# ParaGroup/WindFlow

Hardware: NVIDIA H100
Metric: tuples/sec, Map_GPU->Filter_GPU->Ffat_Windows_GPU (CB win 4096 slide 64) pipeline (higher is better)
Workload: dtype i64+f64

## Files before the change

windflow_b200/csrc/wfb_kernels.cuh:

```cuda
#pragma once
#include <type_traits>
#include <cstdint>
#include <cstring>
#include <cuda.h>
#include <cuda_runtime.h>
#include "wfb_ptx.cuh"
#include "wfb_keys.cuh"

namespace wfb {

template <class P> using key_codec = KeyCodec<typename P::key_t>;
template <class P> using key_words_t = typename key_codec<P>::words_t;
template <class P>
__host__ __device__ __forceinline__ key_words_t<P> key_words(const typename P::tuple_t &t, const typename P::params_t &prm)
{
    return key_codec<P>::encode(P::key(t, prm));
}

constexpr int TILE = 256;
constexpr uint32_t OSW_TILE_POS = 4096;
#ifndef WFB_STAGES
#define WFB_STAGES 4
#endif
constexpr int STAGES = WFB_STAGES;
// ... 410 lines not shown
    auto stage_aux = [&](uint32_t s) { return smem + s * SM::stage_bytes + SM::tile_bytes; };

    if (tid == 0) {
        for (int s = 0; s < SM::stages; s++) { mbar_init(&full[s], 1); mbar_init(&staged[s], TILE / 32); mbar_init(&empty[s], 1); }
        mbar_fence_init();
    }
    if constexpr (MODE == MODE_INGEST) { for (uint32_t i = tid; i < 4u * 256u; i += TP_THREADS) s_hist[i] = 0; }
    __syncthreads();

    if (warp == 0) {
        if (lane == 0) {
            const uint64_t pol_first = l2_policy_evict_first();
            DevBatch b = a.one; uint32_t bi = 0, b_end = 0;
            bool have_batch = false;
            const uint32_t tpt = a.tiles_per_ticket ? a.tiles_per_ticket : 1u;
            uint32_t t_next = 0, t_end = 0, claim = 0;
            for (uint32_t it = 0;; it++) {
                const uint32_t s = it % SM::stages, par = (it / SM::stages) & 1u;
                mbar_wait(&empty[s], par ^ 1u);
                StageMeta &m = meta[s];
                if (t_next == t_end) {
                    claim = atomicAdd(a.ticket, 1u) - a.ticket_base;
                    t_next = claim * tpt;
                    if (claim >= (a.num_tiles + tpt - 1) / tpt) { m.tile = TILE_SENTINEL; mbar_arrive(&full[s]); break; }
                    t_end = min(t_next + tpt, a.num_tiles);
                }
                const uint32_t t = t_next++;
                if (a.batches != nullptr && !(have_batch && t >= b.tile_begin && t < b_end)) {
                    uint32_t lo = 0, hi = a.nbatches - 1;
                    while (lo < hi) { const uint32_t mid = (lo + hi + 1) >> 1; if (a.batches[mid].tile_begin <= t) lo = mid; else hi = mid - 1; }
                    bi = lo; b = a.batches[lo];
                    b_end = (lo + 1 < a.nbatches) ? a.batches[lo + 1].tile_begin : a.num_tiles;
                    have_batch = true;
                }
                const uint32_t first = (t - b.tile_begin) * TILE;
                const uint32_t cnt = min(static_cast<uint32_t>(TILE), b.n - first);
                const unsigned char *src = b.tuples + static_cast<size_t>(first) * TB;
                uint32_t flags = 0, tx = 0;
                const uint64_t off = reinterpret_cast<uint64_t>(src) - a.tmap_base;
                if (CAN_SWZ && a.use_tmap && cnt == TILE && (off & 63u) == 0 && (off >> 6) < 0x7fffff00ull) flags = TF_SWZ;
                else if (!bulk_ok(src, cnt * TB)) flags = TF_FALLBACK;
                if (!(flags & TF_FALLBACK)) tx += cnt * TB;
                const uint64_t *tsp = ((MODE == MODE_FILTER || MODE == MODE_FLATMAP) && b.ts != nullptr) ? b.ts + first : nullptr;
                if (tsp != nullptr && bulk_ok(tsp, cnt * 8u)) { flags |= TF_TS_SMEM; tx += cnt * 8u; }
                if (t_next == t_end) flags |= TF_WIDE_LAST;
                m.tile = t; m.batch = bi; m.first = first; m.cnt = cnt; m.flags = flags; m.wide = claim;
                if (tx) mbar_expect_tx(&full[s], tx); else mbar_arrive(&full[s]);
// ... 545 lines not shown
        if (c.z) atomicAdd(ctl_counts + tid * 4 + 2, c.z);
        if (c.w) atomicAdd(ctl_counts + tid * 4 + 3, c.w);
    }
}

static __global__ void __launch_bounds__(OSW_THREADS) k_wide_chunk_sums16(const uint16_t *__restrict__ H, uint32_t tiles, uint32_t chunk_shift, uint32_t *__restrict__ C,
                                                                          uint32_t *__restrict__ ctl_counts = nullptr)
{
    const uint32_t chunk = blockIdx.x, tid = threadIdx.x;
    const uint32_t t0 = chunk << chunk_shift, t1 = min(tiles, t0 + (1u << chunk_shift));
    uint4 acc = make_uint4(0, 0, 0, 0);
    const ushort4 *row = reinterpret_cast<const ushort4 *>(H) + tid;
#pragma unroll 16
    for (uint32_t t = t0; t < t1; t++) { const ushort4 v = row[static_cast<size_t>(t) * (OSW_DIGITS / 4)]; acc.x += v.x; acc.y += v.y; acc.z += v.z; acc.w += v.w; }
    reinterpret_cast<uint4 *>(C + static_cast<size_t>(chunk) * OSW_DIGITS)[tid] = acc;
    if (ctl_counts != nullptr) {
        if (acc.x) atomicAdd(ctl_counts + tid * 4 + 0, acc.x);
        if (acc.y) atomicAdd(ctl_counts + tid * 4 + 1, acc.y);
        if (acc.z) atomicAdd(ctl_counts + tid * 4 + 2, acc.z);
        if (acc.w) atomicAdd(ctl_counts + tid * 4 + 3, acc.w);
    }
}

static __global__ void __launch_bounds__(OSW_THREADS) k_wide_tile_bases(const uint16_t *__restrict__ H, uint32_t tiles, uint32_t chunk_shift, uint32_t chunks,
                                                                        uint32_t *__restrict__ C, uint32_t *__restrict__ T, uint32_t *__restrict__ ctl_counts,
                                                                        uint32_t *__restrict__ done, uint32_t gshift)
{
    static_assert(OSW_THREADS * 4 == OSW_DIGITS, "four digits per thread");
    constexpr uint32_t NW = OSW_THREADS / 32;
    __shared__ uint32_t wsum[NW];
    __shared__ uint32_t s_last;
    const uint32_t chunk = blockIdx.x, tid = threadIdx.x, lane = tid & 31, warp = tid >> 5;
    const uint32_t t0 = chunk << chunk_shift, t1 = min(tiles, t0 + (1u << chunk_shift));
    uint4 acc = make_uint4(0, 0, 0, 0);
    const ushort4 *row = reinterpret_cast<const ushort4 *>(H) + tid;
    uint4 *trow = reinterpret_cast<uint4 *>(T) + tid;
#pragma unroll 8
    for (uint32_t t = t0; t < t1; t++) {
        const ushort4 v = row[static_cast<size_t>(t) * (OSW_DIGITS / 4)];
        if ((t & ((1u << gshift) - 1u)) == 0) trow[static_cast<size_t>(t >> gshift) * (OSW_DIGITS / 4)] = acc;
        acc.x += v.x; acc.y += v.y; acc.z += v.z; acc.w += v.w;
    }
    uint4 *C4 = reinterpret_cast<uint4 *>(C);
    C4[static_cast<size_t>(chunk) * (OSW_DIGITS / 4) + tid] = acc;
    __threadfence();
    __syncthreads();
    if (tid == 0) s_last = atomicAdd(done, 1u) == chunks - 1u;
    __syncthreads();
    if (!s_last) return;
    __threadfence();
    uint4 tot = make_uint4(0, 0, 0, 0);
#pragma unroll 8
    for (uint32_t c = 0; c < chunks; c++) { const uint4 v = __ldcg(C4 + static_cast<size_t>(c) * (OSW_DIGITS / 4) + tid); tot.x += v.x; tot.y += v.y; tot.z += v.z; tot.w += v.w; }
    reinterpret_cast<uint4 *>(ctl_counts)[tid] = tot;
    const uint32_t sum = tot.x + tot.y + tot.z + tot.w;
    uint32_t incl = sum;
#pragma unroll
    for (int o = 1; o < 32; o <<= 1) { const uint32_t v = __shfl_up_sync(FULL, incl, o); if (lane >= static_cast<uint32_t>(o)) incl += v; }
    if (lane == 31) wsum[warp] = incl;
    __syncthreads();
    uint32_t base = incl - sum;
#pragma unroll
    for (uint32_t q = 0; q < NW; q++) if (q < warp) base += wsum[q];
    uint4 run = make_uint4(base, base + tot.x, base + tot.x + tot.y, base + tot.x + tot.y + tot.z);
#pragma unroll 8
    for (uint32_t c = 0; c < chunks; c++) {
        uint4 *p = C4 + static_cast<size_t>(c) * (OSW_DIGITS / 4) + tid;
        const uint4 v = __ldcg(p);
        *p = run;
        run.x += v.x; run.y += v.y; run.z += v.z; run.w += v.w;
    }
    if (tid == 0) *done = 0;
}

constexpr uint32_t OSR_SMEM = OSR_GROUP_POS * 2u * 2u + OSW_DIGITS * 8u + OSW_DIGITS * 2u;
static_assert(OSR_GROUP == 4 && OSR_GROUP_POS <= 0x8000u, "one ushort4 of part sizes per digit; 16-bit packed position compare");
static __global__ void __launch_bounds__(OSW_THREADS, 3) k_wide_scatter_ranked(const uint32_t *__restrict__ packed, uint32_t *__restrict__ list_out,
                                                                            uint32_t n, uint32_t shift, uint32_t chunk_shift,
                                                                            uint32_t tiles, const uint16_t *__restrict__ H, const uint32_t *__restrict__ Cx,
                                                                            const uint32_t *__restrict__ T)
{
    constexpr uint32_t NW = OSW_THREADS / 32;
    static_assert(OSW_THREADS * 4 == OSW_DIGITS, "four digits per thread");
    extern __shared__ __align__(16) unsigned char osr_smem_buf[];
    uint16_t *lpos = reinterpret_cast<uint16_t *>(osr_smem_buf);
    uint16_t *lslot = lpos + OSR_GROUP_POS;
    ushort4 *part = reinterpret_cast<ushort4 *>(lslot + OSR_GROUP_POS);
    uint16_t *cell = reinterpret_cast<uint16_t *>(part + OSW_DIGITS);
    __shared__ uint32_t wsum[NW];
    __shared__ uint32_t s_total;
    const uint32_t tid = threadIdx.x, lane = tid & 31, warp = tid >> 5, group = blockIdx.x, tile0 = group * OSR_GROUP;
    const uint32_t start = tile0 * OSW_TILE;
    if (start >= n) return;
    {
        ushort4 h[OSR_GROUP];
#pragma unroll
        for (uint32_t k = 0; k < OSR_GROUP; k++)
            h[k] = tile0 + k < tiles ? reinterpret_cast<const ushort4 *>(H)[static_cast<size_t>(tile0 + k) * (OSW_DIGITS / 4) + tid] : make_ushort4(0, 0, 0, 0);
        part[4 * tid + 0] = make_ushort4(h[0].x, h[1].x, h[2].x, h[3].x);
        part[4 * tid + 1] = make_ushort4(h[0].y, h[1].y, h[2].y, h[3].y);
        part[4 * tid + 2] = make_ushort4(h[0].z, h[1].z, h[2].z, h[3].z);
        part[4 * tid + 3] = make_ushort4(h[0].w, h[1].w, h[2].w, h[3].w);
        uint32_t c0 = 0, c1 = 0, c2 = 0, c3 = 0;
#pragma unroll
        for (uint32_t k = 0; k < OSR_GROUP; k++) { c0 += h[k].x; c1 += h[k].y; c2 += h[k].z; c3 += h[k].w; }
        const uint32_t sum = c0 + c1 + c2 + c3;
        uint32_t incl = sum;
#pragma unroll
        for (int o = 1; o < 32; o <<= 1) { const uint32_t v = __shfl_up_sync(FULL, incl, o); if (lane >= static_cast<uint32_t>(o)) incl += v; }
        if (lane == 31) wsum[warp] = incl;
        __syncthreads();
        uint32_t base = incl - sum;
#pragma unroll
        for (uint32_t q = 0; q < NW; q++) if (q < warp) base += wsum[q];
        if (tid == OSW_THREADS - 1) s_total = base + sum;
// ... 44 lines not shown
    }
}

#ifndef WFB_OSR_MINBLOCKS
#define WFB_OSR_MINBLOCKS 6
#endif
template <int RBYTES>
static __global__ void __launch_bounds__(OSW_THREADS, WFB_OSR_MINBLOCKS) k_wide_scatter_ranked_tile(const uint32_t *__restrict__ packed, uint32_t *__restrict__ keys_out,
                                                                            uint32_t list, uint32_t n, uint32_t shift, uint32_t chunk_shift,
                                                                            const uint16_t *__restrict__ H, const uint32_t *__restrict__ Cx, const uint32_t *__restrict__ T,
                                                                            const unsigned char *__restrict__ payload_in, unsigned char *__restrict__ payload_out)
{
    constexpr uint32_t NW = OSW_THREADS / 32;
    constexpr uint32_t LPOS = OSW_TILE + OSW_DIGITS;
    constexpr uint32_t LPAD = 0x0fffu;
    static_assert(OSW_TILE <= 4096 && LPOS % (2 * OSW_THREADS) == 0, "16-bit packed position compare");
    __shared__ __align__(16) uint32_t sw[OSW_TILE];
    __shared__ __align__(16) uint32_t bin_base[OSW_DIGITS];
    __shared__ __align__(8) uint16_t cnt_row[OSW_DIGITS], cell_start[OSW_DIGITS];
    __shared__ __align__(4) uint16_t lpos[LPOS];
    __shared__ uint32_t wsum[NW];
    const uint32_t tid = threadIdx.x, lane = tid & 31, warp = tid >> 5, tile = blockIdx.x;
    const uint32_t start = tile * OSW_TILE;
    if (start >= n) return;
#pragma unroll
    for (uint32_t r = 0; r < OSW_ITEMS; r++) {
        const uint32_t i = r * OSW_THREADS + tid, idx = start + i;
        const uint32_t w = idx < n ? packed[idx] : INVALID_SLOT;
        sw[i] = w;
        if constexpr (RBYTES != 0)
            if (w != INVALID_SLOT) asm volatile("prefetch.global.L2 [%0];" ::"l"(payload_in + static_cast<size_t>(idx) * RBYTES));
    }
    {
        const uint4 cb = reinterpret_cast<const uint4 *>(Cx)[static_cast<size_t>(tile >> chunk_shift) * (OSW_DIGITS / 4) + tid];
        const uint4 tb = reinterpret_cast<const uint4 *>(T)[static_cast<size_t>(tile) * (OSW_DIGITS / 4) + tid];
        reinterpret_cast<uint4 *>(bin_base)[tid] = make_uint4(cb.x + tb.x, cb.y + tb.y, cb.z + tb.z, cb.w + tb.w);
        const ushort4 c = reinterpret_cast<const ushort4 *>(H)[static_cast<size_t>(tile) * (OSW_DIGITS / 4) + tid];
        reinterpret_cast<ushort4 *>(cnt_row)[tid] = c;
        const uint32_t p0 = (c.x + 1u) & ~1u, p1 = (c.y + 1u) & ~1u, p2 = (c.z + 1u) & ~1u, p3 = (c.w + 1u) & ~1u;
        const uint32_t sum = p0 + p1 + p2 + p3;
        uint32_t incl = sum;
#pragma unroll
        for (int o = 1; o < 32; o <<= 1) { const uint32_t v = __shfl_up_sync(FULL, incl, o); if (lane >= static_cast<uint32_t>(o)) incl += v; }
        if (lane == 31) wsum[warp] = incl;
#pragma unroll
        for (uint32_t i = 0; i < LPOS / (2 * OSW_THREADS); i++) reinterpret_cast<uint32_t *>(lpos)[i * OSW_THREADS + tid] = LPAD | (LPAD << 16);
// ... 549 lines not shown
    __shared__ uint32_t s_idx[CAP];
    __shared__ uint32_t s_list[CAP];
    __shared__ __align__(16) uint16_t s_col[BK_KEYS][CS];
    __shared__ uint32_t kcnt[BK_KEYS], koff[BK_KEYS];
    __shared__ uint32_t kleft[BK_KEYS];
    __shared__ uint32_t kcp[BK_KEYS], kleaf[BK_KEYS];
    __shared__ uint64_t kc[BK_KEYS], kg[BK_KEYS], ktt[BK_KEYS];
    __shared__ __align__(16) unsigned char kacc[BK_KEYS * RB];
    __shared__ __align__(16) unsigned char s_sib[LAZY ? 16 : BK_KEYS * BK_SIBL * RB];
    __shared__ uint32_t s_heavy[BK_KEYS];
    __shared__ uint32_t ksegb[BK_KEYS];
    __shared__ uint32_t seg_desc[BK_THREADS];
    __shared__ uint32_t misc[NW], s_boff[2], s_nheavy, s_hnext, s_nseg;

    const uint32_t tid = threadIdx.x, lane = tid & 31, warp = tid >> 5;
    const uint32_t bucket = blockIdx.x;
    const uint32_t kpc = min(BK_KEYS, 1u << shift);
    const uint32_t key_lo = bucket << shift;
    const uint32_t n = ff.n_leaves, logn = ff.log_leaves;
    const uint32_t P32 = static_cast<uint32_t>(ff.pane);
    const uint64_t group_items = ff.slide * ff.nb;
    const size_t tree_stride = static_cast<size_t>(2 * n - 1) * RB;
    BK_TRACE_STATE;

    BK_MARK(0);
    uint32_t my_total = 0;
    uint64_t st_c = 0;
    const bool has_key = tid < kpc && key_lo + tid < ff.max_keys;
    if (has_key) {
        const uint32_t slot = key_lo + tid;
        st_c = ff.cnt[slot];
#pragma unroll
        for (uint32_t q = 0; q < RB / CPB; q++) cp_async<CPB>(kacc + tid * RB + q * CPB, ff.acc + static_cast<size_t>(slot) * RB + q * CPB);
    }
    if (tid < BK_KEYS) kleft[tid] = 0;
    {
        uint32_t cc[DPT];
#pragma unroll
        for (uint32_t q = 0; q < DPT / 4; q++) {
            const uint4 v = reinterpret_cast<const uint4 *>(digit_counts)[tid * (DPT / 4) + q];
            cc[4 * q] = v.x; cc[4 * q + 1] = v.y; cc[4 * q + 2] = v.z; cc[4 * q + 3] = v.w;
        }
        uint32_t sum = 0;
#pragma unroll
        for (uint32_t q = 0; q < DPT; q++) sum += cc[q];
        uint32_t incl = sum;
// ... 373 lines not shown
        uint32_t range = (ws == 0) ? n : (ws & (0u - ws));
        const uint32_t pw = 1u << (31 - __clz(remaining));
        range = min(range, pw);
        const uint32_t level = 31 - __clz(range);
        alignas(16) R node;
        ld_rec<R>(tree + static_cast<size_t>(level_off(n, level) + (ws >> level)) * RB, node);
        P::comb(res, node, res, prm);
        ws = (ws + range) & (n - 1);
        remaining -= range;
    }
    if (opos < out_cap) {
        st_rec<R>(out_res + static_cast<size_t>(opos) * RB, res);
        if (out_ts != nullptr) out_ts[opos] = wm;
    } else atomicOr(ff.err_flags, 2u);
}

template <class P>
__global__ void __launch_bounds__(256) k_ffat_windows(const FfatDev ff, const uint32_t *__restrict__ batch_off,
                                                      const DevBatch *__restrict__ batches, uint32_t nbatches,
                                                      unsigned char *__restrict__ out_res, uint64_t *__restrict__ out_ts, uint32_t out_cap,
                                                      const typename P::params_t prm, uint32_t *__restrict__ n_out)
{
    using R = typename P::result_t;
    if (blockIdx.x == 0 && threadIdx.x == 0 && n_out != nullptr) {
        if (*n_out > out_cap) { *n_out = out_cap; atomicOr(ff.err_flags, 2u); }
        if (ff.results_total != nullptr) *ff.results_total += *n_out;
    }
    const uint32_t nt = min(*ff.n_trig, ff.trig_cap);
    const uint64_t total = static_cast<uint64_t>(nt) * ff.nb;
    const size_t tree_stride = static_cast<size_t>(2 * ff.n_leaves - 1) * sizeof(R);
    for (uint64_t w = blockIdx.x * static_cast<uint64_t>(blockDim.x) + threadIdx.x; w < total; w += static_cast<uint64_t>(gridDim.x) * blockDim.x) {
        const uint32_t ti = static_cast<uint32_t>(w / ff.nb), i = static_cast<uint32_t>(w % ff.nb);
        const Trigger tr = ff.trig[ti];
        const uint64_t wm = batch_watermark(batch_off, batches, nbatches, tr.last_pos);
        ffat_eval_window<P>(ff, ff.tree + static_cast<size_t>(tr.slot) * tree_stride, trig_key<P>(ff, tr), tr.g * ff.nb + i, wm, tr.obase + i,
                            out_res, out_ts, out_cap, prm);
    }
}

template <class P>
__global__ void __launch_bounds__(128) k_ffat_windows_lazy(const FfatDev ff, const uint32_t *__restrict__ batch_off,
                                                           const DevBatch *__restrict__ batches, uint32_t nbatches,
                                                           unsigned char *__restrict__ out_res, uint64_t *__restrict__ out_ts, uint32_t out_cap,
                                                           const typename P::params_t prm, uint32_t *__restrict__ n_out)
{
    using R = typename P::result_t;
    constexpr uint32_t RB = sizeof(R);
    extern __shared__ __align__(16) unsigned char lazy_smem[];
    if (blockIdx.x == 0 && threadIdx.x == 0 && n_out != nullptr) {
        if (*n_out > out_cap) { *n_out = out_cap; atomicOr(ff.err_flags, 2u); }
        if (ff.results_total != nullptr) *ff.results_total += *n_out;
    }
    const uint32_t lane = threadIdx.x & 31, warp = threadIdx.x >> 5, wpb = blockDim.x >> 5;
    const uint32_t n = ff.n_leaves, logn = ff.log_leaves;
    unsigned char *t = lazy_smem + static_cast<size_t>(warp) * 2u * n * RB;
    const uint32_t nt = min(*ff.n_trig, ff.trig_cap);
    const size_t tree_stride = static_cast<size_t>(2 * n - 1) * RB;
    FfatDev fs = ff; fs.lazy = 0;
    for (uint32_t ti = blockIdx.x * wpb + warp; ti < nt; ti += gridDim.x * wpb) {
        const Trigger tr = ff.trig[ti];
        const unsigned char *leaves = ff.tree + static_cast<size_t>(tr.slot) * tree_stride;
        for (uint32_t i = lane; i < n * (RB / 8); i += 32) reinterpret_cast<uint64_t *>(t)[i] = reinterpret_cast<const uint64_t *>(leaves)[i];
        __syncwarp();
        for (uint32_t l = 0; l < logn; l++) {
            const unsigned char *src = t + static_cast<size_t>(level_off(n, l)) * RB;
            unsigned char *dst = t + static_cast<size_t>(level_off(n, l + 1)) * RB;
            for (uint32_t i = lane; i < (n >> (l + 1)); i += 32) {
                alignas(16) R a, b, o;
                ld_rec<R>(src + static_cast<size_t>(2 * i) * RB, a); ld_rec<R>(src + static_cast<size_t>(2 * i + 1) * RB, b);
                o = a;
                P::comb(a, b, o, prm);
// ... 1043 lines not shown
```

windflow_b200/csrc/wfb_launch.cuh:

```cuda
#pragma once
#include <type_traits>
#include <algorithm>
#include <cstring>
#include <cuda.h>
#include <cuda_runtime.h>
#include "../../include/wfb200.h"
#include "wfb_kernels.cuh"

#define WFB_CK(call) do { cudaError_t e__ = (call); if (e__ != cudaSuccess) return static_cast<int>(e__); } while (0)

namespace wfb {

inline int num_sms()
{
    static int n = 0;
    if (n == 0) { int dev = 0; if (cudaGetDevice(&dev) == cudaSuccess) cudaDeviceGetAttribute(&n, cudaDevAttrMultiProcessorCount, dev); }
    return n;
}


typedef CUresult (*PFN_encodeTiled)(CUtensorMap *, CUtensorMapDataType, cuuint32_t, void *, const cuuint64_t *, const cuuint64_t *,
                                    const cuuint32_t *, const cuuint32_t *, CUtensorMapInterleave, CUtensorMapSwizzle,
                                    CUtensorMapL2promotion, CUtensorMapFloatOOBfill);
inline PFN_encodeTiled get_encode_tiled()
{
    static PFN_encodeTiled fn = nullptr;
    static bool tried = false;
    if (!tried) {
        tried = true;
        void *p = nullptr;
        cudaDriverEntryPointQueryResult q;
        if (cudaGetDriverEntryPoint("cuTensorMapEncodeTiled", &p, cudaEnableDefault, &q) == cudaSuccess && q == cudaDriverEntryPointSuccess)
            fn = reinterpret_cast<PFN_encodeTiled>(p);
        cudaGetLastError();
    }
    return fn;
}

inline bool make_tuple_tmap(CUtensorMap *m, uint64_t base, uint64_t end)
{
// ... 114 lines not shown
    }
    return WFB_E_BADARG;
}

template <class P>
int ffat_update_dispatch(const FfatDev &ff, const unsigned char *lifted, const uint32_t *sorted_pos, const uint32_t *batch_off,
                         const DevBatch *batches, uint32_t nbatches, unsigned char *out_res, uint64_t *out_ts,
                         uint32_t out_cap, uint32_t *n_out, uint32_t grid, cudaStream_t s, const void *params, uint32_t lanes_grid)
{
    const typename P::params_t prm = load_params<P>(params);
    k_ffat_update_lanes<P><<<lanes_grid, 128, 0, s>>>(ff, lifted, sorted_pos, batch_off, batches, nbatches, out_res, out_ts, out_cap, n_out, prm);
    k_ffat_update<P><<<std::max(1u, std::min(grid, static_cast<uint32_t>(wfb::num_sms()) * 2u)), 256, 0, s>>>(
        ff, lifted, sorted_pos, batch_off, batches, nbatches, out_res, out_ts, out_cap, n_out, prm);
    WFB_CK(cudaGetLastError());
    return 0;
}

template <class P>
int ffat_buckets_dispatch(const FfatDev &ff, const unsigned char *lifted, const uint32_t *bk_list, uint32_t pos_base,
                          const uint32_t *digit_counts, uint32_t shift, uint32_t moved, const uint32_t *batch_off, const DevBatch *batches,
                          uint32_t nbatches, unsigned char *out_res, uint64_t *out_ts, uint32_t out_cap, uint32_t *n_out, cudaStream_t s,
                          const void *params)
{
    if (ff.lazy) k_ffat_update_buckets<P, true><<<OSW_DIGITS, BK_THREADS, 0, s>>>(ff, lifted, bk_list, pos_base, digit_counts, shift, moved, batch_off, batches,
                                                                                 nbatches, out_res, out_ts, out_cap, n_out, load_params<P>(params));
    else k_ffat_update_buckets<P, false><<<OSW_DIGITS, BK_THREADS, 0, s>>>(ff, lifted, bk_list, pos_base, digit_counts, shift, moved, batch_off, batches,
                                                                          nbatches, out_res, out_ts, out_cap, n_out, load_params<P>(params));
    WFB_CK(cudaGetLastError());
    return 0;
}
template <class P>
constexpr decltype(ProgramOps::ffat_buckets) ffat_buckets_of()
{
    if constexpr (bk_fits<sizeof(typename P::result_t)>()) return &ffat_buckets_dispatch<P>; else return nullptr;
}

template <class P>
int ffat_windows_dispatch(const FfatDev &ff, const uint32_t *batch_off, const DevBatch *batches, uint32_t nbatches,
                          unsigned char *out_res, uint64_t *out_ts, uint32_t out_cap, uint32_t grid, cudaStream_t s, const void *params, uint32_t *n_out)
{
    if (ff.lazy) {
        const size_t per_warp = static_cast<size_t>(2) * ff.n_leaves * sizeof(typename P::result_t);
        const uint32_t wpb = static_cast<uint32_t>(std::max<size_t>(1, std::min<size_t>(4, (32u << 10) / per_warp)));
        k_ffat_windows_lazy<P><<<grid, 32 * wpb, wpb * per_warp, s>>>(ff, batch_off, batches, nbatches, out_res, out_ts, out_cap, load_params<P>(params), n_out);
    } else
    k_ffat_windows<P><<<grid, 256, 0, s>>>(ff, batch_off, batches, nbatches, out_res, out_ts, out_cap, load_params<P>(params), n_out);
    WFB_CK(cudaGetLastError());
    return 0;
}

inline uint32_t grid_for(uint32_t n, uint32_t per_block) { return std::max(1u, std::min((n + per_block - 1) / per_block, static_cast<uint32_t>(wfb::num_sms()) * 16u)); }

template <class P>
int extract_keys_dispatch(const unsigned char *tuples, uint32_t n, uint64_t *keys, uint32_t *dest, uint32_t num_shards, cudaStream_t s,
                          const void *params)
{
    k_extract_keys<P><<<grid_for(n, 256), 256, 0, s>>>(tuples, n, keys, dest, num_shards, load_params<P>(params));
    WFB_CK(cudaGetLastError());
    return 0;
}
template <class P>
int reduce_segments_dispatch(const unsigned char *tuples, const uint64_t *ts, const uint32_t *sidx, const uint32_t *seg_begin,
                             const uint32_t *n_keys, unsigned char *out_tuples, uint64_t *out_ts, uint32_t n, cudaStream_t s,
                             const void *params)
{
    k_reduce_segments<P><<<grid_for(n, 8), 256, 0, s>>>(tuples, ts, sidx, seg_begin, n_keys, out_tuples, out_ts, load_params<P>(params));
    WFB_CK(cudaGetLastError());
    return 0;
}
template <class P>
// ... 246 lines not shown
```

windflow_b200/csrc/wfb_lib.cu:

```cuda
#include <cstdio>
#include <cstdlib>
#include <cstring>
#include <ctime>
#include <mutex>
#include <vector>
#include <algorithm>
#include <atomic>
#include <new>
#include <cuda.h>
#include <cuda_runtime.h>
#include "../../include/wfb200.h"
#include "wfb_kernels.cuh"
#include "wfb_launch.cuh"
#include "wfb_programs.cuh"
#include "wfb_scratch.h"

using namespace wfb;

#define CK(call) do { cudaError_t e__ = (call); if (e__ != cudaSuccess) return static_cast<int>(e__); } while (0)

namespace {

int g_num_sms = 0;

// ... 104 lines not shown
    Scratch<uint64_t> state;
    uint32_t epoch = 0;
    uint64_t launches = 0;

    static constexpr size_t CTL_WORDS = OS_MAX_PASSES * 256 + OS_MAX_PASSES > OSW_DIGITS + 1 ? OS_MAX_PASSES * 256 + OS_MAX_PASSES : OSW_DIGITS + 1;
    static int prepare(uint32_t *ctl_buf, uint32_t passes, cudaStream_t s)
    {
        passes = std::min<uint32_t>(std::max(1u, passes), OS_MAX_PASSES);
        WFB_CK(cudaMemsetAsync(ctl_buf, 0, sizeof(uint32_t) * (passes * 256 + passes), s));
        return 0;
    }

    static int prepare_wide(uint32_t *ctl_buf, cudaStream_t s)
    {
        WFB_CK(cudaMemsetAsync(ctl_buf, 0, sizeof(uint32_t) * (OSW_DIGITS + 1), s));
        return 0;
    }
    Scratch<uint16_t> wideH; Scratch<uint32_t> wideC;
    Scratch<uint32_t> wideT;
    Scratch<uint32_t> wideDone;
    static void wide_geometry(uint32_t cap, bool prefix, uint32_t *tiles, uint32_t *chunk_shift, uint32_t *chunks)
    {
        *tiles = std::max(1u, (cap + OSW_TILE - 1) / OSW_TILE);
        uint32_t cs = prefix ? 5 : 4;
        if (!prefix) while ((1u << (2 * cs)) < *tiles) cs++;
        *chunk_shift = cs;
        *chunks = (*tiles + (1u << cs) - 1) >> cs;
    }
    int ensure_wide_buffers(uint32_t tiles, uint32_t chunks, ScratchWaits waits)
    {
        const size_t rows = static_cast<size_t>(OSW_DIGITS) * tiles, chunk_rows = static_cast<size_t>(OSW_DIGITS) * chunks;
        CK(wideH.ensure(rows, waits, rows));
        CK(wideT.ensure(rows, waits, rows));
        CK(wideC.ensure(chunk_rows, waits, chunk_rows));
        return 0;
    }
    int ensure_wide(uint32_t cap, ScratchWaits waits, uint16_t **rows)
    {
        uint32_t tiles, chunk_shift, chunks;
        wide_geometry(cap, true, &tiles, &chunk_shift, &chunks);
        { int rc = ensure_wide_buffers(tiles, chunks, waits); if (rc) return rc; }
        *rows = wideH;
        return 0;
    }
    template <class K, int RBYTES>
    void launch_wide_scatter(uint32_t tiles, const K *kin, K *kout, uint32_t *vout, const uint32_t *n_ptr, uint32_t n_host, uint32_t shift,
                             uint32_t chunk_shift, const uint32_t *c, cudaStream_t s, const unsigned char *pin, unsigned char *pout, uint32_t pbytes,
                             uint32_t skip_invalid, uint32_t region_stride)
    {
        k_wide_scatter<K, RBYTES><<<tiles, OSW_THREADS, 0, s>>>(kin, kout, vout, n_ptr, n_host, shift, chunk_shift, wideH, wideC, c, pin, pout, pbytes, skip_invalid, region_stride);
    }
    template <class K>
    int sort_wide(const K *kin, K *kout, uint32_t *vout, const uint32_t *n_ptr, uint32_t n_host, uint32_t cap, uint32_t shift,
                  cudaStream_t s, uint32_t *ready_ctl, const uint32_t **counts, const unsigned char *payload_in = nullptr,
                  unsigned char *payload_out = nullptr, uint32_t payload_bytes = 0, bool skip_invalid = false, uint32_t region_stride = 0, uint32_t few_bins = 0,
                  const uint16_t *h16_rows = nullptr, bool list = false)
    {
        if (payload_in && (payload_bytes == 0 || (payload_bytes & 7u))) return WFB_E_BADARG;
        CK(ctl.ensure(CTL_WORDS));
        const bool ranked = ready_ctl && !few_bins;
        const uint16_t *rows = h16_rows ? h16_rows : wideH;
        uint32_t tiles, chunk_shift, chunks;
        wide_geometry(cap, ranked, &tiles, &chunk_shift, &chunks);
        { int rc = ensure_wide_buffers(tiles, chunks, s); if (rc) return rc; }
        uint32_t *c = ready_ctl ? ready_ctl : ctl;
        if (!ready_ctl) { int rc = prepare_wide(c, s); if (rc) return rc; }
        if (ranked) {
            CK(wideDone.ensure_zeroed(1, s));
            k_wide_tile_bases<<<chunks, OSW_THREADS, 0, s>>>(rows, tiles, chunk_shift, chunks, wideC, wideT, c, wideDone,
                                                             osr_group(tiles, payload_in != nullptr) == OSR_GROUP ? 2u : 0u);
        } else if (ready_ctl) {
            k_wide_chunk_sums16<<<chunks, OSW_THREADS, 0, s>>>(rows, tiles, chunk_shift, wideC, c);
        } else {
            CK(cudaMemsetAsync(wideC, 0, sizeof(uint32_t) * OSW_DIGITS * chunks, s));
            k_wide_tile_hist<K><<<tiles, OSW_THREADS, 0, s>>>(kin, n_ptr, n_host, shift, chunk_shift, wideH, wideC, c, skip_invalid ? 1u : 0u);
        }
        if (region_stride && few_bins && payload_in && few_bins <= 32 && (payload_bytes == 16 || payload_bytes == 24 || payload_bytes == 32 || payload_bytes == 64)) {
            const uint32_t *d32 = reinterpret_cast<const uint32_t *>(kin);
            static_assert(sizeof(K) == 4 || sizeof(K) == 8, "key width");
            if (sizeof(K) == 4) {
                switch (payload_bytes) {
                    case 16: k_shard_scatter<16><<<tiles, OSW_THREADS, 0, s>>>(d32, n_host, few_bins, chunk_shift, wideH, wideC, payload_in, payload_out, region_stride); break;
                    case 24: k_shard_scatter<24><<<tiles, OSW_THREADS, 0, s>>>(d32, n_host, few_bins, chunk_shift, wideH, wideC, payload_in, payload_out, region_stride); break;
                    case 32: k_shard_scatter<32><<<tiles, OSW_THREADS, 0, s>>>(d32, n_host, few_bins, chunk_shift, wideH, wideC, payload_in, payload_out, region_stride); break;
                    default: k_shard_scatter<64><<<tiles, OSW_THREADS, 0, s>>>(d32, n_host, few_bins, chunk_shift, wideH, wideC, payload_in, payload_out, region_stride); break;
                }
                CK(cudaGetLastError());
                launches += 2;
                *counts = c;
                return 0;
            }
        }
        if (ranked) {
            if (sizeof(K) != 4 || !kout || (payload_in ? !payload_out || region_stride : !list) || (list && n_host > BKL_RANGE_POS)) return WFB_E_UNSUPPORTED;
            if (!payload_in && osr_group(tiles, false) == OSR_GROUP) {
                CK(osr_smem_attr());
                k_wide_scatter_ranked<<<(tiles + OSR_GROUP - 1) / OSR_GROUP, OSW_THREADS, OSR_SMEM, s>>>(reinterpret_cast<const uint32_t *>(kin), reinterpret_cast<uint32_t *>(kout),
                                                                                                       n_host, shift, chunk_shift, tiles, rows, wideC, wideT);
            }
#define WFB_WSRT(RB_) k_wide_scatter_ranked_tile<RB_><<<tiles, OSW_THREADS, 0, s>>>(reinterpret_cast<const uint32_t *>(kin), reinterpret_cast<uint32_t *>(kout), list ? 1u : 0u, \
                                                                                  n_host, shift, chunk_shift, rows, wideC, wideT, payload_in, payload_out)
            else if (!payload_in) WFB_WSRT(0);
            else switch (payload_bytes) {
                case 16: WFB_WSRT(16); break; case 24: WFB_WSRT(24); break; case 32: WFB_WSRT(32); break; case 48: WFB_WSRT(48); break; case 64: WFB_WSRT(64); break;
                default: return WFB_E_UNSUPPORTED;
            }
#undef WFB_WSRT
            CK(cudaGetLastError());
            launches += 2;
            *counts = c;
            return 0;
        }
#define WFB_WS(RB_) launch_wide_scatter<K, RB_>(tiles, kin, kout, vout, n_ptr, n_host, shift, chunk_shift, c, s, payload_in, payload_out, payload_bytes, skip_invalid ? 1u : 0u, region_stride)
        if (!payload_in) WFB_WS(0);
        else switch (payload_bytes) {
            case 8: WFB_WS(8); break;   case 16: WFB_WS(16); break; case 24: WFB_WS(24); break; case 32: WFB_WS(32); break;
            case 48: WFB_WS(48); break; case 64: WFB_WS(64); break; default: WFB_WS(-1); break;
        }
#undef WFB_WS
        CK(cudaGetLastError());
        launches += 2;
        *counts = c;
        return 0;
    }
// ... 1342 lines not shown
        return 0;
    }
    nbatches = static_cast<uint32_t>(hb.size());
    FfatDev ff;
    const auto ingest = [&]() -> int {
        const bool sparse = h->buckets;
        const uint64_t seg_cap = sparse ? static_cast<uint64_t>(tiles) * TILE : total;
        if (seg_cap > 0x7fffffffull) return WFB_E_BADARG;
        rc = ffat_ensure_segment(h, g, static_cast<uint32_t>(seg_cap), nbatches, s); if (rc) return rc;
        rc = h->ts.ensure_tiles(tiles); if (rc) return rc;
        { int rc_ = h->ts.stage.h2d(g.d_batches, hb.data(), sizeof(DevBatch) * nbatches, s); if (rc_) return rc_; }
        g.nbatches = nbatches; g.total = static_cast<uint32_t>(seg_cap);
        if (sparse) {
            std::vector<uint32_t> boff(nbatches + 1);
            for (uint32_t i = 0; i < nbatches; i++) boff[i] = hb[i].tile_begin * TILE;
            boff[nbatches] = tiles * TILE;
            { int rc_ = h->ts.stage.h2d(g.batch_off, boff.data(), sizeof(uint32_t) * (nbatches + 1), s); if (rc_) return rc_; }
        }

        ff = h->ff;
        ff.seg_cnt = g.seg_cnt; ff.trig = g.trig; ff.n_trig = g.n_trig; ff.trig_cap = static_cast<uint32_t>(g.trig.capacity()); ff.n_heavy = g.n_heavy;

        const uint32_t npasses = h->buckets ? 1u : h->sort_passes;
        rc = h->buckets ? RadixSorter::prepare_wide(g.sort_ctl, s) : RadixSorter::prepare(g.sort_ctl, npasses, s); if (rc) return rc;
        h->mark(0, s);
        TileArgs a; std::memset(&a, 0, sizeof(a));
        a.sort_ctl = g.sort_ctl; a.sort_passes = npasses; a.sort_shift = h->buckets ? h->bucket_shift : 0u; a.sort_dbits = h->buckets ? OSW_BITS : 8u;
        a.batches = g.d_batches; a.nbatches = nbatches; a.num_tiles = tiles;
        a.lifted = g.lifted; a.slots = g.slotsA; a.batch_off = g.batch_off; a.n_total = g.n_total; a.ff = ff;
        g.lifted_src = g.lifted;
        if (sparse && !h->pipelined && !h->bucket_move && (h->ops->reserved & 1u)) {
            const unsigned char *base = hb[0].tuples;
            bool ok = (reinterpret_cast<uintptr_t>(base) & 15u) == 0;
            for (uint32_t i = 0; ok && i < nbatches; i++) ok = hb[i].tuples == base + static_cast<size_t>(hb[i].tile_begin) * TILE * h->ops->tuple_bytes;
            if (ok) { a.inplace = 1; g.lifted_src = base; a.ext_slots = ext_slots; }
        }
        if (ext_slots != nullptr && !a.inplace) {
            if (sparse) return WFB_E_UNSUPPORTED;
            if (nbatches != 1 || !(h->ops->reserved & 1u)) return WFB_E_BADARG;
            a.ext_slots = ext_slots;
        }
        h->ts.next_launch(a);
        a.max_ctas_per_sm = h->pipelined ? 2u : 0u;
        a.l2_hints = 1;
        a.sparse = sparse ? 1u : 0u;
        a.count_keys = h->buckets ? 0u : 1u;
        uint32_t claims = tiles;
// ... 8 lines not shown
            a.tiles_per_ticket = OSW_TILE_POS / TILE;
            a.sort_ctl = nullptr;
            a.pack_rank = 1;
            claims = (tiles + a.tiles_per_ticket - 1) / a.tiles_per_ticket;
        }
        if (a.inplace && h->ops->slots_inplace) {
            rc = h->ops->slots_inplace(a, pre ? static_cast<const void *>(pre) : h->pp(), s); if (rc) return rc;
        } else {
            uint32_t grid = 0;
            rc = h->ops->tile_pass(MODE_INGEST, a, pre ? static_cast<const void *>(pre) : h->pp(), claims, s, &grid, span_begin, span_end); if (rc) return rc;
            h->ts.launched(claims, grid);
        }
        h->launches++;
        h->mark(1, s);
        return 0;
    };
    rc = ingest(); if (rc) return rc;
    for (bool grew = h->ff.grow != 0; grew; ) {
        rc = ffat_grow(h, s, &grew); if (rc) return rc;
        if (grew) { rc = ingest(); if (rc) return rc; h->launches++; }
    }

    if (!h->pipelined) {
        if (!h->append_results) CK(cudaMemsetAsync(n_out_dev, 0, sizeof(uint32_t), s));
        rc = ffat_window_phase(h, g, ff, out, out_ts, out_capacity, n_out_dev, s); if (rc) return rc;
        h->mark(3, s);
    } else {
        CK(cudaEventRecord(g.ev_ingest, s));
        rc = ffat_deliver(h, prev, out, out_ts, out_capacity, n_out_dev, s); if (rc) return rc;
        CK(cudaStreamWaitEvent(h->s2, g.ev_ingest, 0));
        CK(cudaMemsetAsync(g.res_n, 0, sizeof(uint32_t), h->s2));
        rc = ffat_window_phase(h, g, ff, g.res, g.res_ts, static_cast<uint32_t>(g.res_ts.capacity()), g.res_n, h->s2); if (rc) return rc;
        h->mark(3, h->s2);
        CK(cudaEventRecord(g.ev_done, h->s2));
        g.pending = true;
    }
    if (h->timing && h->tev_used < wfb_ffat::TEV_MAX) h->tev_used++;
    h->call_no++;
    return 0;
}

static int ffat_process_prebucketed(wfb_ffat *h, const unsigned char *records, const uint32_t *recv_slots, const uint32_t *bins, uint32_t nsrc,
                                    uint32_t bps, const uint32_t *offs_h, const uint64_t *wms_h, uint32_t slot_mask, uint32_t shift,
                                    void *out_results, uint64_t *out_ts, uint32_t out_capacity, uint32_t *n_out_dev, cudaStream_t s, bool append, uint32_t items)
{
    if (!h || !n_out_dev || nsrc == 0 || nsrc > MAX_SHARDS || bps == 0 || bps > OSW_DIGITS || (1u << shift) > BK_KEYS) return WFB_E_BADARG;
    if (h->win_type != 0 || h->pipelined || !h->buckets) return WFB_E_UNSUPPORTED;
// ... 704 lines not shown
```

windflow_b200/csrc/wfb_ptx.cuh:

```cuda
#pragma once
#include <cstdint>
#include <cuda_runtime.h>

namespace wfb {

__device__ __forceinline__ uint32_t smem_u32(const void *p)
{
    return static_cast<uint32_t>(__cvta_generic_to_shared(p));
}

__device__ __forceinline__ void mbar_init(uint64_t *bar, uint32_t count)
{
    asm volatile("mbarrier.init.shared::cta.b64 [%0], %1;" ::"r"(smem_u32(bar)), "r"(count) : "memory");
}
__device__ __forceinline__ void mbar_fence_init()
{
    asm volatile("fence.mbarrier_init.release.cluster;" ::: "memory");
}
__device__ __forceinline__ void mbar_expect_tx(uint64_t *bar, uint32_t bytes)
{
    asm volatile("mbarrier.arrive.expect_tx.shared::cta.b64 _, [%0], %1;" ::"r"(smem_u32(bar)), "r"(bytes) : "memory");
}
__device__ __forceinline__ bool mbar_try_wait(uint64_t *bar, uint32_t parity)
{
// ... 95 lines not shown
    asm volatile("{\n\t.reg .b128 c, v, d;\n\t"
                 "mov.b128 c, {%2, %3};\n\t"
                 "mov.b128 v, {%4, %5};\n\t"
                 "atom.relaxed.gpu.global.cas.b128 d, [%6], c, v;\n\t"
                 "mov.b128 {%0, %1}, d;\n\t}"
                 : "=l"(old_lo), "=l"(old_hi)
                 : "l"(cmp_lo), "l"(cmp_hi), "l"(val_lo), "l"(val_hi), "l"(p)
                 : "memory");
}

__device__ __forceinline__ uint4 ld_stream_u4(const void *p)
{
    uint4 v;
    asm volatile("ld.global.nc.L1::no_allocate.v4.u32 {%0,%1,%2,%3}, [%4];"
                 : "=r"(v.x), "=r"(v.y), "=r"(v.z), "=r"(v.w) : "l"(p));
    return v;
}
__device__ __forceinline__ void st_stream_u4(void *p, uint4 v)
{
    asm volatile("st.global.L1::no_allocate.v4.u32 [%0], {%1,%2,%3,%4};"
                 ::"l"(p), "r"(v.x), "r"(v.y), "r"(v.z), "r"(v.w) : "memory");
}

__device__ __forceinline__ uint32_t lane_id() { return threadIdx.x & 31u; }
__device__ __forceinline__ uint32_t lanemask_lt()
{
    uint32_t m;
    asm("mov.u32 %0, %%lanemask_lt;" : "=r"(m));
    return m;
}

}
```

Baseline: 17.03 billion.

## Use programmatic dependent launch and split wide-sort base scan into digit slices

Result: faster. 17.52 billion, median of 6 (+2.9%).

```diff
diff --git a/windflow_b200/csrc/wfb_kernels.cuh b/windflow_b200/csrc/wfb_kernels.cuh
--- a/windflow_b200/csrc/wfb_kernels.cuh
+++ b/windflow_b200/csrc/wfb_kernels.cuh
@@ -456,7 +456,10 @@
                 if (t_next == t_end) {
                     claim = atomicAdd(a.ticket, 1u) - a.ticket_base;
                     t_next = claim * tpt;
-                    if (claim >= (a.num_tiles + tpt - 1) / tpt) { m.tile = TILE_SENTINEL; mbar_arrive(&full[s]); break; }
+                    if (claim >= (a.num_tiles + tpt - 1) / tpt) {
+                        griddep_launch_dependents();
+                        m.tile = TILE_SENTINEL; mbar_arrive(&full[s]); break;
+                    }
                     t_end = min(t_next + tpt, a.num_tiles);
                 }
                 const uint32_t t = t_next++;
@@ -1048,55 +1051,92 @@
     }
 }
 
-static __global__ void __launch_bounds__(OSW_THREADS) k_wide_tile_bases(const uint16_t *__restrict__ H, uint32_t tiles, uint32_t chunk_shift, uint32_t chunks,
-                                                                        uint32_t *__restrict__ C, uint32_t *__restrict__ T, uint32_t *__restrict__ ctl_counts,
-                                                                        uint32_t *__restrict__ done, uint32_t gshift)
-{
-    static_assert(OSW_THREADS * 4 == OSW_DIGITS, "four digits per thread");
-    constexpr uint32_t NW = OSW_THREADS / 32;
-    __shared__ uint32_t wsum[NW];
-    __shared__ uint32_t s_last;
-    const uint32_t chunk = blockIdx.x, tid = threadIdx.x, lane = tid & 31, warp = tid >> 5;
-    const uint32_t t0 = chunk << chunk_shift, t1 = min(tiles, t0 + (1u << chunk_shift));
-    uint4 acc = make_uint4(0, 0, 0, 0);
-    const ushort4 *row = reinterpret_cast<const ushort4 *>(H) + tid;
-    uint4 *trow = reinterpret_cast<uint4 *>(T) + tid;
-#pragma unroll 8
-    for (uint32_t t = t0; t < t1; t++) {
-        const ushort4 v = row[static_cast<size_t>(t) * (OSW_DIGITS / 4)];
-        if ((t & ((1u << gshift) - 1u)) == 0) trow[static_cast<size_t>(t >> gshift) * (OSW_DIGITS / 4)] = acc;
-        acc.x += v.x; acc.y += v.y; acc.z += v.z; acc.w += v.w;
-    }
-    uint4 *C4 = reinterpret_cast<uint4 *>(C);
-    C4[static_cast<size_t>(chunk) * (OSW_DIGITS / 4) + tid] = acc;
+constexpr uint32_t WB_SLICES = 8, WB_SLICE_DIGITS = OSW_DIGITS / WB_SLICES, WB_SUB = OSW_THREADS / (WB_SLICE_DIGITS / 4);
+constexpr uint32_t WB_CHUNK_SHIFT = 5, WB_TILES_PER_WARP = (1u << WB_CHUNK_SHIFT) / WB_SUB;
+constexpr uint32_t WB_CTL_WORDS = 2 + 2 * WB_SLICES;
+static_assert(WB_SLICE_DIGITS == 4 * 32 && WB_SUB * 32 == OSW_THREADS && WB_TILES_PER_WARP == OSR_GROUP,
+              "a lane owns 4 digits of the slice; a warp owns WB_TILES_PER_WARP tiles of the chunk, a whole group");
+static __global__ void __launch_bounds__(OSW_THREADS) k_wide_bases(const uint16_t *__restrict__ H, uint32_t tiles, uint32_t chunks,
+                                                                   uint32_t *__restrict__ C, uint32_t *__restrict__ T, uint32_t *__restrict__ ctl_counts,
+                                                                   uint32_t *__restrict__ ctl, uint32_t gshift)
+{
+    __shared__ uint4 part[WB_SUB][32];
+    __shared__ uint32_t s_ticket, s_last, s_base;
+    const uint32_t tid = threadIdx.x, lane = tid & 31, warp = tid >> 5;
+    griddep_wait();
+    if (tid == 0) s_ticket = atomicAdd(ctl, 1u);
+    __syncthreads();
+    const uint32_t slice = s_ticket / chunks, chunk = s_ticket % chunks;
+    const size_t dq = slice * (WB_SLICE_DIGITS / 4) + lane;
+    uint4 *C4 = reinterpret_cast<uint4 *>(C), *T4 = reinterpret_cast<uint4 *>(T);
+    {
+        const uint32_t t0 = (chunk << WB_CHUNK_SHIFT) + warp * WB_TILES_PER_WARP;
+        ushort4 v[WB_TILES_PER_WARP];
+#pragma unroll
+        for (uint32_t k = 0; k < WB_TILES_PER_WARP; k++)
+            v[k] = t0 + k < tiles ? reinterpret_cast<const ushort4 *>(H)[static_cast<size_t>(t0 + k) * (OSW_DIGITS / 4) + dq] : make_ushort4(0, 0, 0, 0);
+        uint4 s = make_uint4(0, 0, 0, 0);
+#pragma unroll
+        for (uint32_t k = 0; k < WB_TILES_PER_WARP; k++) { s.x += v[k].x; s.y += v[k].y; s.z += v[k].z; s.w += v[k].w; }
+        part[warp][lane] = s;
+        __syncthreads();
+        uint4 acc = make_uint4(0, 0, 0, 0);
+#pragma unroll
+        for (uint32_t w = 0; w < WB_SUB; w++)
+            if (w < warp) { const uint4 p = part[w][lane]; acc.x += p.x; acc.y += p.y; acc.z += p.z; acc.w += p.w; }
+#pragma unroll
+        for (uint32_t k = 0; k < WB_TILES_PER_WARP; k++) {
+            const uint32_t t = t0 + k;
+            if (t < tiles && (t & ((1u << gshift) - 1u)) == 0) T4[static_cast<size_t>(t >> gshift) * (OSW_DIGITS / 4) + dq] = acc;
+            acc.x += v[k].x; acc.y += v[k].y; acc.z += v[k].z; acc.w += v[k].w;
+        }
+        if (warp == WB_SUB - 1) C4[static_cast<size_t>(chunk) * (OSW_DIGITS / 4) + dq] = acc;
+    }
     __threadfence();
     __syncthreads();
-    if (tid == 0) s_last = atomicAdd(done, 1u) == chunks - 1u;
+    if (tid == 0) s_last = atomicAdd(ctl + 2 + slice, 1u) == chunks - 1u;
     __syncthreads();
     if (!s_last) return;
     __threadfence();
-    uint4 tot = make_uint4(0, 0, 0, 0);
+    const uint32_t K = (chunks + WB_SUB - 1) / WB_SUB, c0 = min(chunks, warp * K), c1 = min(chunks, c0 + K);
+    uint4 s = make_uint4(0, 0, 0, 0);
 #pragma unroll 8
-    for (uint32_t c = 0; c < chunks; c++) { const uint4 v = __ldcg(C4 + static_cast<size_t>(c) * (OSW_DIGITS / 4) + tid); tot.x += v.x; tot.y += v.y; tot.z += v.z; tot.w += v.w; }
-    reinterpret_cast<uint4 *>(ctl_counts)[tid] = tot;
+    for (uint32_t c = c0; c < c1; c++) { const uint4 p = __ldcg(C4 + static_cast<size_t>(c) * (OSW_DIGITS / 4) + dq); s.x += p.x; s.y += p.y; s.z += p.z; s.w += p.w; }
+    part[warp][lane] = s;
+    __syncthreads();
+    uint4 run = make_uint4(0, 0, 0, 0), tot = make_uint4(0, 0, 0, 0);
+#pragma unroll
+    for (uint32_t w = 0; w < WB_SUB; w++) {
+        const uint4 p = part[w][lane];
+        if (w < warp) { run.x += p.x; run.y += p.y; run.z += p.z; run.w += p.w; }
+        tot.x += p.x; tot.y += p.y; tot.z += p.z; tot.w += p.w;
+    }
     const uint32_t sum = tot.x + tot.y + tot.z + tot.w;
     uint32_t incl = sum;
 #pragma unroll
     for (int o = 1; o < 32; o <<= 1) { const uint32_t v = __shfl_up_sync(FULL, incl, o); if (lane >= static_cast<uint32_t>(o)) incl += v; }
-    if (lane == 31) wsum[warp] = incl;
-    __syncthreads();
-    uint32_t base = incl - sum;
-#pragma unroll
-    for (uint32_t q = 0; q < NW; q++) if (q < warp) base += wsum[q];
-    uint4 run = make_uint4(base, base + tot.x, base + tot.x + tot.y, base + tot.x + tot.y + tot.z);
+    uint32_t *published = ctl + 2 + WB_SLICES;
+    if (tid == 31) st_release_u32(published + slice, incl + 1u);
+    if (warp == 0) {
+        uint32_t before = 0;
+        if (lane < slice) { uint32_t p; while ((p = ld_acquire_u32(published + lane)) == 0) { } before = p - 1u; }
+#pragma unroll
+        for (int o = 16; o > 0; o >>= 1) before += __shfl_xor_sync(FULL, before, o);
+        if (lane == 0) s_base = before;
+    }
+    if (warp == 0) reinterpret_cast<uint4 *>(ctl_counts)[dq] = tot;
+    __syncthreads();
+    const uint32_t base = s_base + incl - sum;
+    run.x += base; run.y += base + tot.x; run.z += base + tot.x + tot.y; run.w += base + tot.x + tot.y + tot.z;
 #pragma unroll 8
-    for (uint32_t c = 0; c < chunks; c++) {
-        uint4 *p = C4 + static_cast<size_t>(c) * (OSW_DIGITS / 4) + tid;
+    for (uint32_t c = c0; c < c1; c++) {
+        uint4 *p = C4 + static_cast<size_t>(c) * (OSW_DIGITS / 4) + dq;
         const uint4 v = __ldcg(p);
         *p = run;
         run.x += v.x; run.y += v.y; run.z += v.z; run.w += v.w;
     }
-    if (tid == 0) *done = 0;
+    if (tid == 0 && atomicAdd(ctl + 1, 1u) == WB_SLICES - 1u)
+        for (uint32_t i = 0; i < WB_CTL_WORDS; i++) ctl[i] = 0;
 }
 
 constexpr uint32_t OSR_SMEM = OSR_GROUP_POS * 2u * 2u + OSW_DIGITS * 8u + OSW_DIGITS * 2u;
@@ -1117,6 +1157,7 @@
     __shared__ uint32_t s_total;
     const uint32_t tid = threadIdx.x, lane = tid & 31, warp = tid >> 5, group = blockIdx.x, tile0 = group * OSR_GROUP;
     const uint32_t start = tile0 * OSW_TILE;
+    griddep_wait();
     if (start >= n) return;
     {
         ushort4 h[OSR_GROUP];
@@ -1207,6 +1248,7 @@
     __shared__ uint32_t wsum[NW];
     const uint32_t tid = threadIdx.x, lane = tid & 31, warp = tid >> 5, tile = blockIdx.x;
     const uint32_t start = tile * OSW_TILE;
+    griddep_wait();
     if (start >= n) return;
 #pragma unroll
     for (uint32_t r = 0; r < OSW_ITEMS; r++) {
@@ -1802,6 +1844,7 @@
     const uint64_t group_items = ff.slide * ff.nb;
     const size_t tree_stride = static_cast<size_t>(2 * n - 1) * RB;
     BK_TRACE_STATE;
+    griddep_wait();
 
     BK_MARK(0);
     uint32_t my_total = 0;
@@ -2221,6 +2264,7 @@
                                                       const typename P::params_t prm, uint32_t *__restrict__ n_out)
 {
     using R = typename P::result_t;
+    griddep_wait();
     if (blockIdx.x == 0 && threadIdx.x == 0 && n_out != nullptr) {
         if (*n_out > out_cap) { *n_out = out_cap; atomicOr(ff.err_flags, 2u); }
         if (ff.results_total != nullptr) *ff.results_total += *n_out;
@@ -2246,6 +2290,7 @@
     using R = typename P::result_t;
     constexpr uint32_t RB = sizeof(R);
     extern __shared__ __align__(16) unsigned char lazy_smem[];
+    griddep_wait();
     if (blockIdx.x == 0 && threadIdx.x == 0 && n_out != nullptr) {
         if (*n_out > out_cap) { *n_out = out_cap; atomicOr(ff.err_flags, 2u); }
         if (ff.results_total != nullptr) *ff.results_total += *n_out;
diff --git a/windflow_b200/csrc/wfb_launch.cuh b/windflow_b200/csrc/wfb_launch.cuh
--- a/windflow_b200/csrc/wfb_launch.cuh
+++ b/windflow_b200/csrc/wfb_launch.cuh
@@ -2,6 +2,7 @@
 #include <type_traits>
 #include <algorithm>
 #include <cstring>
+#include <utility>
 #include <cuda.h>
 #include <cuda_runtime.h>
 #include "../../include/wfb200.h"
@@ -16,6 +17,18 @@
     static int n = 0;
     if (n == 0) { int dev = 0; if (cudaGetDevice(&dev) == cudaSuccess) cudaDeviceGetAttribute(&n, cudaDevAttrMultiProcessorCount, dev); }
     return n;
+}
+
+template <class... KArgs, class... Args>
+inline cudaError_t launch_pdl(void (*k)(KArgs...), dim3 grid, dim3 block, size_t smem, cudaStream_t s, Args &&...args)
+{
+    cudaLaunchAttribute attr[1];
+    attr[0].id = cudaLaunchAttributeProgrammaticStreamSerialization;
+    attr[0].val.programmaticStreamSerializationAllowed = 1;
+    cudaLaunchConfig_t cfg = {};
+    cfg.gridDim = grid; cfg.blockDim = block; cfg.dynamicSmemBytes = smem; cfg.stream = s;
+    cfg.attrs = attr; cfg.numAttrs = 1;
+    return cudaLaunchKernelEx(&cfg, k, std::forward<Args>(args)...);
 }
 
 
@@ -176,11 +189,8 @@
                           uint32_t nbatches, unsigned char *out_res, uint64_t *out_ts, uint32_t out_cap, uint32_t *n_out, cudaStream_t s,
                           const void *params)
 {
-    if (ff.lazy) k_ffat_update_buckets<P, true><<<OSW_DIGITS, BK_THREADS, 0, s>>>(ff, lifted, bk_list, pos_base, digit_counts, shift, moved, batch_off, batches,
-                                                                                 nbatches, out_res, out_ts, out_cap, n_out, load_params<P>(params));
-    else k_ffat_update_buckets<P, false><<<OSW_DIGITS, BK_THREADS, 0, s>>>(ff, lifted, bk_list, pos_base, digit_counts, shift, moved, batch_off, batches,
-                                                                          nbatches, out_res, out_ts, out_cap, n_out, load_params<P>(params));
-    WFB_CK(cudaGetLastError());
+    WFB_CK(launch_pdl(ff.lazy ? k_ffat_update_buckets<P, true> : k_ffat_update_buckets<P, false>, dim3(OSW_DIGITS), dim3(BK_THREADS), 0, s, ff, lifted, bk_list,
+                      pos_base, digit_counts, shift, moved, batch_off, batches, nbatches, out_res, out_ts, out_cap, n_out, load_params<P>(params)));
     return 0;
 }
 template <class P>
@@ -196,10 +206,10 @@
     if (ff.lazy) {
         const size_t per_warp = static_cast<size_t>(2) * ff.n_leaves * sizeof(typename P::result_t);
         const uint32_t wpb = static_cast<uint32_t>(std::max<size_t>(1, std::min<size_t>(4, (32u << 10) / per_warp)));
-        k_ffat_windows_lazy<P><<<grid, 32 * wpb, wpb * per_warp, s>>>(ff, batch_off, batches, nbatches, out_res, out_ts, out_cap, load_params<P>(params), n_out);
+        WFB_CK(launch_pdl(k_ffat_windows_lazy<P>, dim3(grid), dim3(32 * wpb), wpb * per_warp, s, ff, batch_off, batches, nbatches, out_res, out_ts, out_cap,
+                          load_params<P>(params), n_out));
     } else
-    k_ffat_windows<P><<<grid, 256, 0, s>>>(ff, batch_off, batches, nbatches, out_res, out_ts, out_cap, load_params<P>(params), n_out);
-    WFB_CK(cudaGetLastError());
+    WFB_CK(launch_pdl(k_ffat_windows<P>, dim3(grid), dim3(256), 0, s, ff, batch_off, batches, nbatches, out_res, out_ts, out_cap, load_params<P>(params), n_out));
     return 0;
 }
 
diff --git a/windflow_b200/csrc/wfb_lib.cu b/windflow_b200/csrc/wfb_lib.cu
--- a/windflow_b200/csrc/wfb_lib.cu
+++ b/windflow_b200/csrc/wfb_lib.cu
@@ -150,7 +150,7 @@
     static void wide_geometry(uint32_t cap, bool prefix, uint32_t *tiles, uint32_t *chunk_shift, uint32_t *chunks)
     {
         *tiles = std::max(1u, (cap + OSW_TILE - 1) / OSW_TILE);
-        uint32_t cs = prefix ? 5 : 4;
+        uint32_t cs = prefix ? WB_CHUNK_SHIFT : 4;
         if (!prefix) while ((1u << (2 * cs)) < *tiles) cs++;
         *chunk_shift = cs;
         *chunks = (*tiles + (1u << cs) - 1) >> cs;
@@ -194,9 +194,10 @@
         uint32_t *c = ready_ctl ? ready_ctl : ctl;
         if (!ready_ctl) { int rc = prepare_wide(c, s); if (rc) return rc; }
         if (ranked) {
-            CK(wideDone.ensure_zeroed(1, s));
-            k_wide_tile_bases<<<chunks, OSW_THREADS, 0, s>>>(rows, tiles, chunk_shift, chunks, wideC, wideT, c, wideDone,
-                                                             osr_group(tiles, payload_in != nullptr) == OSR_GROUP ? 2u : 0u);
+            CK(wideDone.ensure_zeroed(WB_CTL_WORDS, s));
+            CK(launch_pdl(k_wide_bases, dim3(WB_SLICES * chunks), dim3(OSW_THREADS), 0, s, rows, tiles, chunks, static_cast<uint32_t *>(wideC),
+                          static_cast<uint32_t *>(wideT), c, static_cast<uint32_t *>(wideDone),
+                          osr_group(tiles, payload_in != nullptr) == OSR_GROUP ? 2u : 0u));
         } else if (ready_ctl) {
             k_wide_chunk_sums16<<<chunks, OSW_THREADS, 0, s>>>(rows, tiles, chunk_shift, wideC, c);
         } else {
@@ -223,11 +224,13 @@
             if (sizeof(K) != 4 || !kout || (payload_in ? !payload_out || region_stride : !list) || (list && n_host > BKL_RANGE_POS)) return WFB_E_UNSUPPORTED;
             if (!payload_in && osr_group(tiles, false) == OSR_GROUP) {
                 CK(osr_smem_attr());
-                k_wide_scatter_ranked<<<(tiles + OSR_GROUP - 1) / OSR_GROUP, OSW_THREADS, OSR_SMEM, s>>>(reinterpret_cast<const uint32_t *>(kin), reinterpret_cast<uint32_t *>(kout),
-                                                                                                       n_host, shift, chunk_shift, tiles, rows, wideC, wideT);
+                CK(launch_pdl(k_wide_scatter_ranked, dim3((tiles + OSR_GROUP - 1) / OSR_GROUP), dim3(OSW_THREADS), OSR_SMEM, s, reinterpret_cast<const uint32_t *>(kin),
+                              reinterpret_cast<uint32_t *>(kout), n_host, shift, chunk_shift, tiles, rows, static_cast<const uint32_t *>(wideC),
+                              static_cast<const uint32_t *>(wideT)));
             }
-#define WFB_WSRT(RB_) k_wide_scatter_ranked_tile<RB_><<<tiles, OSW_THREADS, 0, s>>>(reinterpret_cast<const uint32_t *>(kin), reinterpret_cast<uint32_t *>(kout), list ? 1u : 0u, \
-                                                                                  n_host, shift, chunk_shift, rows, wideC, wideT, payload_in, payload_out)
+#define WFB_WSRT(RB_) CK(launch_pdl(k_wide_scatter_ranked_tile<RB_>, dim3(tiles), dim3(OSW_THREADS), 0, s, reinterpret_cast<const uint32_t *>(kin), \
+                                    reinterpret_cast<uint32_t *>(kout), list ? 1u : 0u, n_host, shift, chunk_shift, rows, static_cast<const uint32_t *>(wideC), \
+                                    static_cast<const uint32_t *>(wideT), payload_in, payload_out))
             else if (!payload_in) WFB_WSRT(0);
             else switch (payload_bytes) {
                 case 16: WFB_WSRT(16); break; case 24: WFB_WSRT(24); break; case 32: WFB_WSRT(32); break; case 48: WFB_WSRT(48); break; case 64: WFB_WSRT(64); break;
@@ -1616,7 +1619,8 @@
         ff.seg_cnt = g.seg_cnt; ff.trig = g.trig; ff.n_trig = g.n_trig; ff.trig_cap = static_cast<uint32_t>(g.trig.capacity()); ff.n_heavy = g.n_heavy;
 
         const uint32_t npasses = h->buckets ? 1u : h->sort_passes;
-        rc = h->buckets ? RadixSorter::prepare_wide(g.sort_ctl, s) : RadixSorter::prepare(g.sort_ctl, npasses, s); if (rc) return rc;
+        if (!h->buckets) { rc = RadixSorter::prepare(g.sort_ctl, npasses, s); if (rc) return rc; }
+        if (!h->pipelined && !h->append_results) CK(cudaMemsetAsync(n_out_dev, 0, sizeof(uint32_t), s));
         h->mark(0, s);
         TileArgs a; std::memset(&a, 0, sizeof(a));
         a.sort_ctl = g.sort_ctl; a.sort_passes = npasses; a.sort_shift = h->buckets ? h->bucket_shift : 0u; a.sort_dbits = h->buckets ? OSW_BITS : 8u;
@@ -1671,7 +1675,6 @@
     }
 
     if (!h->pipelined) {
-        if (!h->append_results) CK(cudaMemsetAsync(n_out_dev, 0, sizeof(uint32_t), s));
         rc = ffat_window_phase(h, g, ff, out, out_ts, out_capacity, n_out_dev, s); if (rc) return rc;
         h->mark(3, s);
     } else {
diff --git a/windflow_b200/csrc/wfb_ptx.cuh b/windflow_b200/csrc/wfb_ptx.cuh
--- a/windflow_b200/csrc/wfb_ptx.cuh
+++ b/windflow_b200/csrc/wfb_ptx.cuh
@@ -141,6 +141,19 @@
                  ::"l"(p), "r"(v.x), "r"(v.y), "r"(v.z), "r"(v.w) : "memory");
 }
 
+__device__ __forceinline__ void griddep_wait()
+{
+#if defined(__CUDA_ARCH__) && __CUDA_ARCH__ >= 900
+    asm volatile("griddepcontrol.wait;" ::: "memory");
+#endif
+}
+__device__ __forceinline__ void griddep_launch_dependents()
+{
+#if defined(__CUDA_ARCH__) && __CUDA_ARCH__ >= 900
+    asm volatile("griddepcontrol.launch_dependents;" ::: "memory");
+#endif
+}
+
 __device__ __forceinline__ uint32_t lane_id() { return threadIdx.x & 31u; }
 __device__ __forceinline__ uint32_t lanemask_lt()
 {
```
